# jovoy/SolarAxionRayTracing

Measured on AMD Instinct MI355X. Metric: rays/sec, higher is better.
Workload: dtype f64

## Files before the change

### solaraxionraytracing_amd/csrc/sart_api.hip

```cpp
#include <hip/hip_runtime.h>
#include <rccl/rccl.h>
#include <dlfcn.h>
#include <sys/mman.h>
#include <unistd.h>

#include <algorithm>
#include <atomic>
#include <cmath>
#include <condition_variable>
#include <thread>
#include <cstdio>
#include <cstdlib>
#include <cstring>
#include <limits>
#include <map>
#include <mutex>
#include <string>
#include <vector>

#include "../../include/sart.h"
#include "sart_device.h"

namespace sart {
void launch_trace_histogram(const HotA& H, const HotB& HB, const DevBlob* blob, const TraceArgs& A, double* acc, int n_blocks,
// ... 45 lines not shown
                            hipStream_t stream);
int records_block();
int compact_chunk_max();
void launch_compact_records(const sart_axion_t* rec, uint32_t n, sart_axion_t* out, unsigned long long capacity, uint32_t* block_counts,
                            unsigned long long* block_first, unsigned long long* counts, hipStream_t stream);
void launch_stage_columns(const HotA& H, const HotB& HB, const DevBlob* blob, const TraceArgs& A, uint64_t* stage, uint32_t* flags,
                          uint32_t mask, int n_blocks, hipStream_t stream);
void launch_compact_columns(const uint64_t* stage, const uint32_t* flags, uint32_t n, uint32_t mask, unsigned long long ray_id0, uint64_t* out,
                            unsigned long long capacity, uint32_t* block_counts, unsigned long long* block_first,
                            unsigned long long* counts, hipStream_t stream);
int histogram_blocks_per_cu(int variant);
void launch_build_solar_tables(const double* em_dev, const double* radii_dev, const double* energies_dev, int n_radii, int n_energies,
                               double* cdf_dev, double* row_sum_dev, double* rcdf_dev, uint16_t* rguide_dev, uint16_t* eguide_dev,
                               uint32_t* status_dev, hipStream_t stream);
void launch_cdf_hi32(const double* cdf_dev, uint32_t* out_dev, size_t n, hipStream_t stream);
}

using namespace sart;

namespace {

thread_local std::string g_err;
int fail(int code, const std::string& msg) {
  g_err = msg;
  return code;
}
#define SART_HIP(call)                                                                              \
  do {                                                                                              \
    hipError_t e_ = (call);                                                                         \
    if (e_ != hipSuccess)                                                                           \
      return fail(e_ == hipErrorOutOfMemory ? SART_ERR_OUT_OF_MEMORY : SART_ERR_NO_DEVICE,          \
                  std::string(#call) + ": " + hipGetErrorString(e_));                               \
  } while (0)

constexpr double kPi = 3.14159265358979323846;
// ... 86 lines not shown
#endif
    bool no_early_reject = false;
    bool no_sure_miss = false;
    bool no_image_tile = false;
    bool no_path_const = false;
    bool no_host_prefault = false;
    int records_chunk = 0;
    int records_fail_chunk = 0;
    int prefault_threads = 0;
    bool force_generic = false;
    int image_replicas = 0;
    int hist_blocks_per_cu = 0;
    bool no_radial_table = false;
    int image_tile_max = 0;
    int a0_wide = 1;
  } knobs;
  double a0_wide_survival = -1.0;
  bool a0_wide_on = false;
  hipStream_t own_stream = nullptr;
  hipStream_t stream = nullptr;
  std::string device_name;

  bool have_setup = false, have_solar = false, have_refl = false, have_det = false;
  sart_setup_t setup;
  std::vector<double> energies;
  int n_radii = 0, n_energies = 0;
  std::vector<double> refl_data;
  int refl_nc = 0, refl_na = 0, refl_ne = 0;
  double refl_amin = 0, refl_amax = 0, refl_emin = 0, refl_emax = 0;
  std::vector<double> sb_x, sb_y, win_x, win_y, gas_x, gas_y;
// ... 3 lines not shown
  HotB hotb;
  DevBuf<DevBlob> d_blob;
  bool blob_dirty = true;
  bool spot_may_have_moved = true;
  std::vector<ShellDev> shells;
  std::vector<uint8_t> shell_lut;
  int radial_n = 0;
  int radius_span = 0;
  bool path_const = false;
  DevBuf<ShellDev> d_shells;
  DevBuf<double> d_sincos;
  DevBuf<uint8_t> d_lut;
  DevBuf<double> d_rcdf, d_ecdf, d_refl;
  DevBuf<uint32_t> d_ecdf_hi32;
  DevBuf<uint16_t> d_rguide, d_eguide;
  DevBuf<EnergyDev> d_etab;
  DevBuf<double> d_replicas;
  DevBuf<double> d_partials;
  DevBuf<double> d_acc;
  bool d_acc_stale = false;
  DevBuf<sart_axion_t> d_rec;
  DevBuf<sart_axion_t> d_rec2;
  DevBuf<sart_axion_t> d_cmp;
  DevBuf<uint32_t> d_cmp_counts;
  DevBuf<unsigned long long> d_cmp_first, d_cmp_totals;
  unsigned long long* h_cmp_totals = nullptr;
  DevBuf<uint64_t> d_col_stage, d_col_cmp[2];
  DevBuf<uint32_t> d_col_flags;
  hipStream_t copy_stream = nullptr;
  hipEvent_t rec_traced[2] = {nullptr, nullptr}, rec_copied[2] = {nullptr, nullptr};
// ... 666 lines not shown
  DevBlob b;
  std::memset(&b, 0, sizeof b);
  b.P = c->params;
  b.T = tables_of(c);
  if (int rc = c->d_blob.upload(&b, 1)) return rc;
  c->hot = hot_of(c->params);
  c->hot.radial_table = radial_table ? 1 : 0;
  c->hotb.diff_flux_cdfs = c->d_ecdf.p;
  c->hotb.cdf_hi32 = c->d_ecdf_hi32.p;
  c->hotb.energy_guide = c->d_eguide.p;
  c->hotb.energy_tab = c->d_etab.p;
  c->hotb.refl = c->d_refl.p;
  c->hotb.n_energies = c->n_energies;
  c->hotb.refl_n_angles = c->refl_na;
  c->hotb.cdf_stride = c->n_energies + kEnergyCdfPad;
  c->hotb._pad = 0;
  if (!c->knobs.no_early_reject) build_zones(c->setup, c->params, c->n_radii, c->hot, tilt_bound_of(c->setup, c->setup.telescope_turned_y_deg));
  if (c->hot.n_zones > 0 && c->knobs.a0_wide > 0) {
    const double survival = a0_survival_of(c->hot);
    if (survival != c->a0_wide_survival) {
      c->a0_wide_survival = survival;
      c->a0_wide_on = a0_wide_rule(survival);
    }
    if (c->knobs.a0_wide == 2 || c->a0_wide_on) c->hot.zone_reached |= kA0WideMask;
  }
  c->path_const = path_is_constant(c->params, c->hot, c->n_radii);
  c->blob_dirty = false;
  if (c->spot_may_have_moved) c->tile.valid = false;
  c->spot_may_have_moved = false;
  return 0;
}
// ... 274 lines not shown
#endif
    c->knobs.no_early_reject = flag("SART_NO_EARLY_REJECT");
    c->knobs.no_sure_miss = flag("SART_NO_SURE_MISS");
    c->knobs.no_image_tile = flag("SART_NO_IMAGE_TILE");
    c->knobs.no_path_const = flag("SART_NO_PATH_CONST");
    c->knobs.no_host_prefault = flag("SART_NO_HOST_PREFAULT");
    c->knobs.records_chunk = number("SART_RECORDS_CHUNK");
    c->knobs.records_fail_chunk = number("SART_RECORDS_FAIL_CHUNK");
    c->knobs.prefault_threads = number("SART_PREFAULT_THREADS");
    c->knobs.force_generic = flag("SART_FORCE_GENERIC");
    c->knobs.image_replicas = number("SART_IMAGE_REPLICAS");
    c->knobs.hist_blocks_per_cu = number("SART_HIST_BLOCKS_PER_CU");
    c->knobs.no_radial_table = flag("SART_NO_RADIAL_TABLE");
    c->knobs.image_tile_max = number("SART_IMAGE_TILE_MAX");
    if (const char* e = std::getenv("SART_A0_WIDE")) c->knobs.a0_wide = std::min(2, std::max(0, std::atoi(e)));
  }
  *out = c;
  return 0;
}

int sart_destroy(sart_context* c) {
  if (!c) return 0;
  (void)hipSetDevice(c->device);
  (void)hipStreamSynchronize(c->stream);
  for (auto& ev : c->events) { (void)hipEventDestroy(ev.first); (void)hipEventDestroy(ev.second); }
  for (int k = 0; k < 2; ++k) {
    if (c->rec_traced[k]) (void)hipEventDestroy(c->rec_traced[k]);
    if (c->rec_copied[k]) (void)hipEventDestroy(c->rec_copied[k]);
  }
  if (c->copy_stream) { (void)hipStreamSynchronize(c->copy_stream); (void)hipStreamDestroy(c->copy_stream); }
// ... 93 lines not shown
  c->spot_may_have_moved = true;
  return hoist_setup(c);
}

int sart_set_axion_mass(sart_context* c, double m) {
  if (!c) return fail(SART_ERR_INVALID_ARGUMENT, "ctx is NULL");
  if (!c->have_setup) return fail(SART_ERR_NOT_READY, "no setup");
  if (!std::isfinite(m)) return fail(SART_ERR_INVALID_ARGUMENT, "axion mass is not finite");
  c->setup.m_axion = m;
  if (c->derived_dirty) return 0;
  c->params.gas_dm2_abs = std::fabs(c->params.gas_m_gamma_sq - m * m);
  c->blob_dirty = true;
  return 0;
}

int sart_set_solar_tables(sart_context* c, const double* rcdf, const double* ecdf, const double* energies, int32_t nR,
                          int32_t nE) {
  if (!c || !rcdf || !ecdf || !energies) return fail(SART_ERR_INVALID_ARGUMENT, "NULL argument");
  if (nR < 1 || nR > 2048) return fail(SART_ERR_INVALID_ARGUMENT, "n_radii must be in [1, 2048] (LDS-resident radius CDF)");
  if (nE < 2 || nE > 65535) return fail(SART_ERR_INVALID_ARGUMENT, "n_energies must be in [2, 65535]");
  for (int i = 1; i < nR; ++i) if (rcdf[i] < rcdf[i - 1]) return fail(SART_ERR_INVALID_ARGUMENT, "flux_radius_cdf not monotone");
  if (rcdf[nR - 1] != 1.0) return fail(SART_ERR_INVALID_ARGUMENT, "flux_radius_cdf must end at 1.0");
  SART_HIP(hipSetDevice(c->device));
  SART_HIP(hipStreamSynchronize(c->stream));
  std::vector<uint16_t> rg(kRadiusGuideEntries);
  for (int k = 0; k < kRadiusGuideEntries; ++k) {
    const double edge = k <= kRadiusGuide ? static_cast<double>(k) / kRadiusGuide
                                          : 0.96875 + static_cast<double>(k - (kRadiusGuide + 1)) / 32768.0;
    rg[k] = static_cast<uint16_t>(std::min<size_t>(lower_bound_idx(rcdf, nR, edge), nR - 1));
  }
// ... 23 lines not shown
      const double edge = 1.0 - decode(kEnergyGuideCode0 - static_cast<uint32_t>(j) + 1u);
      const size_t ub = static_cast<size_t>(std::upper_bound(row, row + nE, edge) - row);
      g[kEnergyGuideUniform + j] = static_cast<uint16_t>(std::min(ub, last));
    }
    g[kEnergyGuideBuckets] = static_cast<uint16_t>(last);
    std::memcpy(padded.data() + static_cast<size_t>(r) * stride, row, static_cast<size_t>(nE) * sizeof(double));
  }
  if (int rc = c->d_rcdf.upload(rcdf, nR)) return rc;
  if (int rc = c->d_ecdf.upload(padded.data(), padded.size())) return rc;
  if (int rc = c->d_ecdf_hi32.resize(padded.size())) return rc;
  launch_cdf_hi32(c->d_ecdf.p, c->d_ecdf_hi32.p, padded.size(), c->stream);
  SART_HIP(hipGetLastError());
  SART_HIP(hipStreamSynchronize(c->stream));
  if (int rc = c->d_rguide.upload(rg.data(), rg.size())) return rc;
  if (int rc = c->d_eguide.upload(eg.data(), eg.size())) return rc;
  c->energies.assign(energies, energies + nE);
  c->n_radii = nR;
  c->n_energies = nE;
  c->have_solar = true;
  c->have_channels = false;
  c->derived_dirty = true;
  return 0;
}

int sart_set_solar_tables_device(sart_context* c, const double* em_rates_dev, const double* radii, const double* energies,
                                 int32_t nR, int32_t nE) {
  if (!c || !em_rates_dev || !radii || !energies) return fail(SART_ERR_INVALID_ARGUMENT, "NULL argument");
  if (nR < 1 || nR > 2048) return fail(SART_ERR_INVALID_ARGUMENT, "n_radii must be in [1, 2048] (LDS-resident radius CDF)");
  if (nE < 2 || nE > 65535) return fail(SART_ERR_INVALID_ARGUMENT, "n_energies must be in [2, 65535]");
  SART_HIP(hipSetDevice(c->device));
// ... 9 lines not shown
  if (int rc = c->d_rguide.resize(kRadiusGuideEntries)) return rc;
  if (int rc = c->d_eguide.resize(static_cast<size_t>(nR) * kEnergyGuideEntries)) return rc;
  if (int rc = c->d_ecdf_hi32.resize(static_cast<size_t>(nR) * (static_cast<size_t>(nE) + kEnergyCdfPad))) return rc;
  c->have_solar = false;
  c->have_channels = false;
  launch_build_solar_tables(em_rates_dev, d_radii.p, d_energies.p, nR, nE, c->d_ecdf.p, d_row_sum.p, c->d_rcdf.p, c->d_rguide.p,
                            c->d_eguide.p, d_status.p, c->stream);
  launch_cdf_hi32(c->d_ecdf.p, c->d_ecdf_hi32.p, c->d_ecdf_hi32.n, c->stream);
  SART_HIP(hipGetLastError());
  uint32_t status[2] = {0, 0};
  SART_HIP(hipMemcpyAsync(status, d_status.p, sizeof status, hipMemcpyDeviceToHost, c->stream));
  SART_HIP(hipStreamSynchronize(c->stream));
  if (status[0] & 1u) return fail(SART_ERR_INVALID_ARGUMENT, "emission table: a radius row does not give a CDF (negative / non-finite rates, or a row that sums to zero)");
  if (status[0] & 2u) return fail(SART_ERR_INVALID_ARGUMENT, "emission table: fluxRadiusCDF is not monotone or does not end at 1.0");
  c->radius_span = static_cast<int>(status[1]);
  c->energies.assign(energies, energies + nE);
  c->n_radii = nR;
  c->n_energies = nE;
  c->have_solar = true;
  c->derived_dirty = true;
  return 0;
}

static_assert(kEnergyGuideEntries == 2594 && kRadiusGuideEntries == 3074, "include/sart.h (sart_get_solar_tables) and _lib.py (ENERGY_GUIDE_ENTRIES, RADIUS_GUIDE_ENTRIES) state these numbers");
int sart_get_solar_tables(sart_context* c, double* rcdf_out, double* ecdf_out, uint16_t* radius_guide_out, uint16_t* energy_guide_out) {
  if (!c) return fail(SART_ERR_INVALID_ARGUMENT, "ctx is NULL");
  if (!c->have_solar) return fail(SART_ERR_NOT_READY, "no solar tables");
  SART_HIP(hipSetDevice(c->device));
  SART_HIP(hipStreamSynchronize(c->stream));
  const size_t nR = static_cast<size_t>(c->n_radii), nE = static_cast<size_t>(c->n_energies);
// ... 66 lines not shown
__attribute__((visibility("default"))) int sart_internal_zones(sart_context* c, uint32_t* lo, uint32_t* hi, uint32_t* reached_bits) {
  if (!c || !lo || !hi || !reached_bits) return -1;
  if (hipSetDevice(c->device) != hipSuccess || refresh_derived(c) != 0 || sync_blob(c) != 0) return -1;
  for (int z = 0; z < c->hot.n_zones; ++z) { lo[z] = c->hot.zone_lo[z]; hi[z] = c->hot.zone_hi[z]; }
  *reached_bits = c->hot.zone_reached & ((1u << kMaxZones) - 1u);
  return c->hot.n_zones;
}

__attribute__((visibility("default"))) double sart_internal_a0_wide_share(double survival) { return a0_wide_fallback_share(survival); }
__attribute__((visibility("default"))) int sart_internal_a0_wide_rule(double survival) { return a0_wide_rule(survival) ? 1 : 0; }
__attribute__((visibility("default"))) int sart_internal_a0_wide(sart_context* c, double* survival) {
  if (!c || !survival) return -1;
  if (hipSetDevice(c->device) != hipSuccess || refresh_derived(c) != 0 || sync_blob(c) != 0) return -1;
  *survival = c->hot.n_zones > 0 ? a0_survival_of(c->hot) : 1.0;
  return (c->hot.zone_reached >> kA0WideBit) & 1u;
}

__attribute__((visibility("default"))) int sart_internal_shell0_miss_radius(sart_context* c, double* out) {
  if (!c || !out) return fail(SART_ERR_INVALID_ARGUMENT, "NULL argument");
  SART_HIP(hipSetDevice(c->device));
  if (int rc = refresh_derived(c)) return rc;
  if (int rc = sync_blob(c)) return rc;
  *out = c->params.shell0_miss_radius;
  return 0;
}

__attribute__((visibility("default"))) int sart_internal_mirror_miss(sart_context* c, const sart_trace_params_t* params, double* radius,
                                                                     double* slope_sq, double* thresholds, unsigned long long* counts) {
  if (!c || !radius || !slope_sq) return fail(SART_ERR_INVALID_ARGUMENT, "NULL argument");
  SART_HIP(hipSetDevice(c->device));
// ... 1827 lines not shown
```

### solaraxionraytracing_amd/csrc/sart_device.h

```cpp
#pragma once
#include <stdint.h>

namespace sart {

constexpr int kMaxShells = 64;
constexpr int kMaxStrips = 16;
constexpr int kRadiusGuide = 2048;
constexpr int kRadiusGuideTop = 1024;
constexpr uint32_t kRadiusGuideTopStart = 0xF8000000u;
constexpr int kRadiusGuideEntries = kRadiusGuide + 1 + kRadiusGuideTop + 1;
#ifndef SART_ENERGY_GUIDE_DIV
#define SART_ENERGY_GUIDE_DIV 1024
#endif
constexpr int kEnergyGuideDiv = SART_ENERGY_GUIDE_DIV;
constexpr int kEnergyGuideUniform = kEnergyGuideDiv / 32 * 31;
constexpr int kEnergyGuideLogMax = 25 * 64;
constexpr int kEnergyGuideBuckets = kEnergyGuideUniform + kEnergyGuideLogMax + 1;
constexpr int kEnergyGuideEntries = kEnergyGuideBuckets + 1;
constexpr uint32_t kEnergyGuideCode0 = (1023u - 5u) << 6;
constexpr int kEnergyCdfPad = 4;
constexpr int kShellLutMax = 1024;
constexpr int kMaxRadii = 2048;
constexpr int kSinCosEntries = 129;

struct ShellDev {
  double r1;
  double r1_outer;
  double m1_k, m1_hb, m1_cc, m1_zhi;
  double m2_k, m2_hb, m2_cc, m2_zlo, m2_zhi;
  double m2_rc;
  double n1_tan;
  double n1_r3t;
  double n1_r3sq, n1_e;
  double n2_tan;
// ... 74 lines not shown
  uint32_t zone_reached;
  uint32_t zone_lo[4], zone_hi[4];
};
constexpr int kMaxZones = 4;
constexpr int kA0WideBit = 8;
constexpr uint32_t kA0WideMask = 0x5u << kA0WideBit;
static_assert(kA0WideBit >= kMaxZones, "the wide-pass switch lies above the zones' bits");

struct HotB {
  const double* diff_flux_cdfs;
  const uint32_t* cdf_hi32;
  const uint16_t* energy_guide;
  const EnergyDev* energy_tab;
  const double* refl;
  int32_t n_energies, refl_n_angles;
  int32_t cdf_stride, _pad;
};

struct DevTables {
  const double* sincos_tab;
  const ShellDev* shells;
  const uint8_t* shell_lut;
  const double* flux_radius_cdf;
  const uint16_t* radius_guide;
  const double* diff_flux_cdfs;
  const uint16_t* energy_guide;
  const EnergyDev* energy_tab;
  const double* refl;
};

struct DevBlob {
// ... 157 lines not shown
```

### solaraxionraytracing_amd/csrc/sart_kernels.hip

```cpp
#include <hip/hip_runtime.h>
#include <stdint.h>
#include <string.h>

#include <type_traits>

#include "../../include/sart.h"
#include "sart_device.h"
#include "sart_math.h"

namespace sart {

struct U4 { uint32_t x, y, z, w; };
constexpr int kPhiloxRounds = 7;

__device__ __forceinline__ U4 philox4x32(uint32_t c0, uint32_t c1, uint32_t c2, uint32_t c3, uint32_t k0,
                                         uint32_t k1) {
#pragma unroll
  for (int r = 0; r < kPhiloxRounds; ++r) {
    const uint64_t p0 = (uint64_t)0xD2511F53u * c0;
    const uint64_t p1 = (uint64_t)0xCD9E8D57u * c2;
    const uint32_t hi0 = (uint32_t)(p0 >> 32), lo0 = (uint32_t)p0;
    const uint32_t hi1 = (uint32_t)(p1 >> 32), lo1 = (uint32_t)p1;
    const uint32_t n0 = __builtin_amdgcn_bitop3_b32(hi1, c1, k0, 0x96);
    const uint32_t n2 = __builtin_amdgcn_bitop3_b32(hi0, c3, k1, 0x96);
// ... 333 lines not shown
template <typename T>
__device__ __forceinline__ T gload(const void* base, uint32_t byte_off) {
  typedef const __attribute__((address_space(1))) char* gbytes;
  return *reinterpret_cast<const __attribute__((address_space(1))) T*>((gbytes)base + byte_off);
}

typedef uint32_t u4v __attribute__((ext_vector_type(4)));
struct EnergyDraw {
  double u;
  uint32_t khi;
  uint32_t row;
  uint32_t gword;
  uint32_t lo, hi;
  u4v c;
};
template <bool WORD = false>
__device__ __forceinline__ void energy_draw_begin(const HotB& HB, int r_idx, double u5, uint32_t word, EnergyDraw& d, int r_idx_guide = -1) {
  if (r_idx_guide < 0) r_idx_guide = r_idx;
  d.u = u5;
  if (WORD) {
    d.khi = word;
  } else {
    const double w = fmin(u5 + 1.0, 1.9999999999999998);
    d.khi = __builtin_amdgcn_alignbit((uint32_t)__double2hiint(w), (uint32_t)__double2loint(w), 20u);
  }
  static_assert((kEnergyGuideDiv & (kEnergyGuideDiv - 1)) == 0 && kEnergyGuideDiv >= 32, "the word form shifts by log2 of it");
  const double v = 1.0 - u5;
  const uint32_t ku = WORD ? word >> (32 - __builtin_ctz((uint32_t)kEnergyGuideDiv)) : (uint32_t)(int)(u5 * (double)kEnergyGuideDiv);
  const uint32_t code = (uint32_t)__double2hiint(v) >> 14;
  const uint32_t kl = (uint32_t)kEnergyGuideUniform + min(kEnergyGuideCode0 - code, (uint32_t)kEnergyGuideLogMax);
  const bool uniform_bucket = WORD ? word < 0xF8000000u : v > 0.03125;
  const uint32_t k = uniform_bucket ? ku : kl;
  d.row = __umul24((uint32_t)r_idx, (uint32_t)HB.cdf_stride);
  d.gword = gload<uint32_t>(HB.energy_guide, (__umul24((uint32_t)r_idx_guide, (uint32_t)kEnergyGuideEntries) + k) * 2u);
}
__device__ __forceinline__ void energy_draw_candidates(const HotB& HB, EnergyDraw& d) {
  d.lo = d.gword & 0xFFFFu;
  d.hi = d.gword >> 16;
  d.c = gload<u4v>(HB.cdf_hi32, (d.row + d.lo) * 4u);
}
template <bool WORD = false>
__device__ __forceinline__ int energy_draw_finish(const HotB& HB, const EnergyDraw& d) {
  const double u = d.u;
  if (WORD) {
    const uint32_t z = d.khi;
    uint32_t lo = d.lo + (uint32_t)(d.c.x < z) + (uint32_t)(d.c.y < z) + (uint32_t)(d.c.z < z) + (uint32_t)(d.c.w < z);
    if ((d.c.w < z) & (d.hi > d.lo + 4u)) {
      asm volatile("; rare: energy bucket wider than four entries");
      uint32_t hi = d.hi;
      while (lo < hi) {
        const uint32_t mid = (lo + hi) >> 1;
        if (gload<double>(HB.diff_flux_cdfs, (d.row + mid) * 8u) < u) lo = mid + 1; else hi = mid;
      }
    }
    return (int)min(lo, (uint32_t)(HB.n_energies - 1));
  }
  const uint32_t km1 = max(d.khi, 1u) - 1u;
  uint32_t lo = d.lo + (uint32_t)(d.c.x < km1) + (uint32_t)(d.c.y < km1) + (uint32_t)(d.c.z < km1) + (uint32_t)(d.c.w < km1);
// ... 1 lines not shown
  if (((d.c.w < km1) & (d.hi > d.lo + 4u)) | tie) {
    asm volatile("; rare: energy bucket wider than four entries, or a tie in the upper 32 bits");
    if (tie) lo = d.lo;
    uint32_t hi = d.hi;
    while (lo < hi) {
      const uint32_t mid = (lo + hi) >> 1;
      if (gload<double>(HB.diff_flux_cdfs, (d.row + mid) * 8u) < u) lo = mid + 1; else hi = mid;
    }
  }
  return (int)min(lo, (uint32_t)(HB.n_energies - 1));
}
template <bool WORD = false>
__device__ __forceinline__ int sample_energy_index(const HotB& HB, int r_idx, double u5, uint32_t word = 0u) {
  EnergyDraw d;
  energy_draw_begin<WORD>(HB, r_idx, u5, word, d);
  energy_draw_candidates(HB, d);
  return energy_draw_finish<WORD>(HB, d);
}

static_assert(sizeof(EnergyDev) == 8 * sizeof(double), "EnergyDev is loaded as eight f64");
__device__ __forceinline__ EnergyDev load_energy_row(const HotB& HB, int e_idx) {
  const uint32_t off = (uint32_t)e_idx * 64u;
  return EnergyDev{gload<double>(HB.energy_tab, off), gload<double>(HB.energy_tab, off + 8u), gload<double>(HB.energy_tab, off + 16u),
                   gload<double>(HB.energy_tab, off + 24u), gload<double>(HB.energy_tab, off + 32u), gload<double>(HB.energy_tab, off + 40u),
                   gload<double>(HB.energy_tab, off + 48u), gload<double>(HB.energy_tab, off + 56u)};
}

__device__ __forceinline__ double spoke_measure(int n, double c) {
  if (n == 16) {
    const double u = HORNER(c, c, -0.5);
    const double v = HORNER(u, u, -0.125);
// ... 416 lines not shown
  uint64_t m_chip;
  uint64_t m_strip;
};
template <bool RECORDS, bool FAST, int GAS, bool ZEXT, bool SCAN = false, bool NODRAW = false, bool ESCAN = false>
__device__ __forceinline__ void phase_b(const DevParams& P, const LdsTables& L, const HotB& HB, const TraceArgs& A,
                                        const RayState& st, int e_idx_in, bool live, RayOut& out, sart_axion_t* rec,
                                        EScanGeo* geo = nullptr) {
#ifdef SART_STAGE_TIMING
#define SART_B_STAMP(k, dep) do { asm volatile("" :: "v"(dep)); out.tb[k] = __builtin_readcyclecounter(); } while (0)
#else
#define SART_B_STAMP(k, dep)
#endif
  SART_B_STAMP(0, st.X0);
  constexpr bool WORD = !RECORDS;
  const bool draw_energy = NODRAW ? false : __builtin_amdgcn_readfirstlane(e_idx_in) < 0;
  EnergyDraw ed = {};
#ifdef SART_DEBUG_KNOBS
  const uint32_t dbg = (uint32_t)__builtin_amdgcn_readfirstlane((int)A.flags);
  if (draw_energy) energy_draw_begin<WORD>(HB, (dbg & 0x02000000u) ? (st.r_idx & 15) : st.r_idx, st.u5, st.u5_hi, ed, (dbg & 0x04000000u) ? (st.r_idx & 15) : st.r_idx);
#else
  if (draw_energy) energy_draw_begin<WORD>(HB, st.r_idx, st.u5, st.u5_hi, ed);
#endif
  const ShellDev& sh = L.shells[st.shell];
  const int wolter = __builtin_amdgcn_readfirstlane(P.telescope_wolter);
  static_assert(!ZEXT || GAS >= 0, "the z-extent form needs the stage at compile time");
  static_assert(!SCAN || !RECORDS, "the mass scan accumulates, it writes no records");
  const int stage_gas = (GAS >= 0) ? GAS : __builtin_amdgcn_readfirstlane(P.stage_gas);
  const int test_active = FAST ? 0 : __builtin_amdgcn_readfirstlane(P.test_active);
  const int n_half_strips = __builtin_amdgcn_readfirstlane(P.n_half_strips);
  const uint32_t flags = (uint32_t)__builtin_amdgcn_readfirstlane((int)A.flags);
  const double X0 = st.X0, Y0 = st.Y0, tsx = st.tsx, tsy = st.tsy, zcb = st.zcb;
  const double Q0 = fma(X0, X0, Y0 * Y0);

  const double D0 = fma(X0, tsx, Y0 * tsy);
  const double A0 = fma(tsx, tsx, tsy * tsy);
  const double L0 = 1.0 + A0;
  double z1;
  uint64_t live_m = ballot64(live), hit1_m, hit2_m;
  const bool hit1 = pick_root(A0 - sh.m1_k, D0 + sh.m1_hb, Q0 - sh.m1_cc, 0.0, sh.m1_zhi, z1, hit1_m);
  if (!hit1) z1 = zcb;
  const double m1x = fma(z1, tsx, X0), m1y = fma(z1, tsy, Y0);
  double n1z = wolter ? sh.n1_r3t : sh.n1_tan * fma(-sh.n1_tan, z1, sh.r1);
  if (live & !hit1)
    n1z = normal_z_general(P, sh, 1, m1x, m1y, z1);
  if (draw_energy) energy_draw_candidates(HB, ed);
  double wx = tsx, wy = tsy, wz = 1.0;
  const double N1 = fma(m1x, m1x, fma(m1y, m1y, n1z * n1z));
  double sin_a1, sin_a2;
  const double sin2_a1 = reflect(wx, wy, wz, L0, m1x, m1y, n1z, N1, sin_a1);

  {
    const double lz = P.l_mirror - z1, num = sh.nickel_num;
    bool nick = sin2_a1 * fma(lz, lz, num * num) > num * num;
    uint64_t nick_m = ballot64(nick);
    if (ballot64(!(lz > 0.0))) {
      if (!(lz > 0.0)) nick = fsqrt(sin2_a1 / (1.0 - sin2_a1)) > num / lz;
      nick_m = ballot64(nick);
    }
    const bool upper = st.shell > 0;
    const bool hit_nickel = live & upper & nick;
// ... 591 lines not shown
      }
      const int packed = Q.w[wave].idx[slot];
      st.r_idx = packed & 0xFFFF;
      st.shell = packed >> 16;
      if constexpr (kAperture) {
        typename BD::Args APl;
        reload_kernarg(APl, BD::kArgsOffset);
        const double fx = (st.X0 - APl.x_min) * APl.inv_step_x;
        const double fy = (st.Y0 - APl.y_min) * APl.inv_step_y;
        const bool in_window = (fx >= 0.0) & (fx < (double)APl.nx) & (fy >= 0.0) & (fy < (double)APl.ny);
        ap_cell = in_window ? (uint32_t)(int)fy * (uint32_t)APl.nx + (uint32_t)(int)fx : (uint32_t)APl.nx * (uint32_t)APl.ny;
      }
      const DevBlob& Bo = lds_opaque(B);
      HotB HB;
      reload_kernarg(HB, offsetof(HistKernArgs, HB));
      asm volatile("" :: "s"(HB.cdf_hi32), "s"(HB.energy_guide), "s"(HB.energy_tab), "s"(HB.refl), "s"(HB.refl_n_angles), "s"(HB.cdf_stride));
      phase_b<false, false, -1, false>(Bo.P, L, HB, lds_opaque(Ab), st, H.test_active ? Pb.n_energies : -1, valid, out, nullptr);
    }
    h1 += n_valid;
    __builtin_amdgcn_s_setprio(SART_PRIO_ACC);
    n_nickel += (uint32_t)__popcll(out.m_nickel);
    n_till += (uint32_t)__popcll(out.m_till);
    n_passed += (uint32_t)__popcll(out.m_passed);
    [[maybe_unused]] const uint32_t sh = shell_of(st.shell);
    if constexpr (kShells) {
      if (__builtin_amdgcn_inverse_ballot_w64(out.m_nickel))
        __hip_atomic_fetch_add(&lds.tab.cnt[sh][1], 1u, __ATOMIC_RELAXED, __HIP_MEMORY_SCOPE_WORKGROUP);
      if (__builtin_amdgcn_inverse_ballot_w64(out.m_till))
        __hip_atomic_fetch_add(&lds.tab.cnt[sh][2], 1u, __ATOMIC_RELAXED, __HIP_MEMORY_SCOPE_WORKGROUP);
    }
    if (out.passed) {
// ... 1626 lines not shown
  double *d_in = nullptr, *d_out = nullptr, *d_tab = nullptr;
  if (n < 1 || (fn >= 15 && fn <= 20 && (n & 1)) || hipMalloc(&d_in, (size_t)n * 8) != hipSuccess || hipMalloc(&d_out, (size_t)n * 8) != hipSuccess ||
      hipMalloc(&d_tab, 2 * kSinCosEntries * 8) != hipSuccess)
    return -1;
  (void)hipMemcpy(d_in, in_host, (size_t)n * 8, hipMemcpyHostToDevice);
  (void)hipMemcpy(d_tab, sincos_table_host, 2 * kSinCosEntries * 8, hipMemcpyHostToDevice);
  hipLaunchKernelGGL(math_eval_kernel, dim3((n + 255) / 256), dim3(256), 0, nullptr, fn, d_in, d_out, n, d_tab);
  const hipError_t e = hipMemcpy(out_host, d_out, (size_t)n * 8, hipMemcpyDeviceToHost);
  (void)hipFree(d_in); (void)hipFree(d_out); (void)hipFree(d_tab);
  return e == hipSuccess ? 0 : -2;
}

void launch_cdf_hi32(const double* cdf_dev, uint32_t* out_dev, size_t n, hipStream_t stream);
void launch_build_guides(const double* ecdf_dev, int n_rows, int n_energies, uint16_t* eguide_dev, const double* rcdf_dev, int n_radii,
                         uint16_t* rguide_dev, uint32_t* status_dev, hipStream_t stream);
__global__ __launch_bounds__(256) void word_draw_energy_kernel(HotB HB, const int32_t* __restrict__ rows, const uint32_t* __restrict__ words, int n,
                                                               int32_t* __restrict__ out_word, int32_t* __restrict__ out_general) {
  const int i = blockIdx.x * blockDim.x + threadIdx.x;
  if (i >= n) return;
  const uint32_t z = words[i];
  const double u = u52(z, 0u);
  out_word[i] = sample_energy_index<true>(HB, rows[i], u, z);
  out_general[i] = sample_energy_index<false>(HB, rows[i], u);
}
__global__ __launch_bounds__(256) void word_draw_radius_kernel(const double* __restrict__ rcdf, const uint16_t* __restrict__ rguide,
                                                               const double* __restrict__ sincos_tab, int n_radii,
                                                               const uint32_t* __restrict__ words, int n, int32_t* __restrict__ out_word,
                                                               int32_t* __restrict__ out_general) {
  __shared__ TablesLds S;
  DevParams P = {};
  P.n_radii = n_radii;
  DevTables T = {};
  T.sincos_tab = sincos_tab;
  T.flux_radius_cdf = rcdf;
  T.radius_guide = rguide;
  stage_tables<256>(S, P, T);
  const LdsTables L{S.sincos, S.rcdf_hi, rcdf, S.rguide, S.shells, S.lut};
  const int i = blockIdx.x * blockDim.x + threadIdx.x;
  if (i >= n) return;
  const uint32_t z = words[i];
  out_word[i] = radius_draw<true>(L, z, u52(z, 0u));
  out_general[i] = radius_draw<false>(L, z, u52(z, 0u));
}
extern "C" __attribute__((visibility("default"))) int sart_internal_word_draw(int kind, const double* cdf_host, int n_rows, int n_cols,
                                                                               const int32_t* rows_host, const uint32_t* words_host, int n,
                                                                               int32_t* out_word_host, int32_t* out_general_host) {
  if (n < 1 || n_rows < 1 || n_cols < 1 || (kind != 0 && kind != 1) || (kind == 1 && (n_rows != 1 || n_cols > kMaxRadii)) || n_cols > 65535)
    return -1;
  if (kind == 0)
    for (int i = 0; i < n; ++i)
      if (rows_host[i] < 0 || rows_host[i] >= n_rows) return -1;
  const int stride = kind == 0 ? n_cols + kEnergyCdfPad : n_cols;
  std::vector<double> cdf((size_t)n_rows * stride, 1.0);
  for (int r = 0; r < n_rows; ++r)
    for (int k = 0; k < n_cols; ++k) cdf[(size_t)r * stride + k] = cdf_host[(size_t)r * n_cols + k];
  const size_t n_guide = kind == 0 ? (size_t)n_rows * kEnergyGuideEntries : (size_t)kRadiusGuideEntries;
  double *d_cdf = nullptr, *d_tab = nullptr;
  uint32_t *d_hi = nullptr, *d_words = nullptr, *d_status = nullptr;
  uint16_t* d_guide = nullptr;
  int32_t *d_rows = nullptr, *d_ow = nullptr, *d_og = nullptr;
  int rc = -2;
  if (hipMalloc(&d_cdf, cdf.size() * 8) == hipSuccess && hipMalloc(&d_hi, cdf.size() * 4) == hipSuccess &&
      hipMalloc(&d_guide, n_guide * 2) == hipSuccess && hipMalloc(&d_words, (size_t)n * 4) == hipSuccess &&
      hipMalloc(&d_rows, (size_t)n * 4) == hipSuccess && hipMalloc(&d_ow, (size_t)n * 4) == hipSuccess &&
      hipMalloc(&d_og, (size_t)n * 4) == hipSuccess && hipMalloc(&d_status, 8) == hipSuccess &&
      hipMalloc(&d_tab, 2 * kSinCosEntries * 8) == hipSuccess) {
    (void)hipMemcpy(d_cdf, cdf.data(), cdf.size() * 8, hipMemcpyHostToDevice);
    (void)hipMemcpy(d_words, words_host, (size_t)n * 4, hipMemcpyHostToDevice);
    (void)hipMemset(d_rows, 0, (size_t)n * 4);
    (void)hipMemset(d_tab, 0, 2 * kSinCosEntries * 8);
    if (kind == 0) {
      (void)hipMemcpy(d_rows, rows_host, (size_t)n * 4, hipMemcpyHostToDevice);
      launch_cdf_hi32(d_cdf, d_hi, cdf.size(), nullptr);
      launch_build_guides(d_cdf, n_rows, n_cols, d_guide, nullptr, 0, nullptr, d_status, nullptr);
      HotB HB = {};
      HB.diff_flux_cdfs = d_cdf;
      HB.cdf_hi32 = d_hi;
      HB.energy_guide = d_guide;
      HB.n_energies = n_cols;
      HB.cdf_stride = stride;
      hipLaunchKernelGGL(word_draw_energy_kernel, dim3((n + 255) / 256), dim3(256), 0, nullptr, HB, d_rows, d_words, n, d_ow, d_og);
    } else {
      launch_build_guides(nullptr, 0, 0, nullptr, d_cdf, n_cols, d_guide, d_status, nullptr);
      hipLaunchKernelGGL(word_draw_radius_kernel, dim3((n + 255) / 256), dim3(256), 0, nullptr, d_cdf, d_guide, d_tab, n_cols, d_words, n, d_ow,
                         d_og);
    }
    const hipError_t e1 = hipMemcpy(out_word_host, d_ow, (size_t)n * 4, hipMemcpyDeviceToHost);
    const hipError_t e2 = hipMemcpy(out_general_host, d_og, (size_t)n * 4, hipMemcpyDeviceToHost);
    rc = (e1 == hipSuccess && e2 == hipSuccess && hipGetLastError() == hipSuccess) ? 0 : -2;
  }
  (void)hipFree(d_cdf); (void)hipFree(d_hi); (void)hipFree(d_guide); (void)hipFree(d_words); (void)hipFree(d_rows);
  (void)hipFree(d_ow); (void)hipFree(d_og); (void)hipFree(d_status); (void)hipFree(d_tab);
  return rc;
}

int records_block() { return kRecBlock; }
int histogram_block_of(int) { return 1024; }

#define SART_HIST_VARIANTS(X) \
  X(0, true, false, 0, false) X(1, false, false, -1, false) X(2, false, true, -1, false) X(3, true, false, 1, false) \
  X(4, true, true, 0, false) X(5, true, false, 0, true) X(6, true, false, 1, true)
#define SART_SCAN_VARIANTS(X) X(1, false, false, -1, false) X(2, false, true, -1, false) X(3, true, false, 1, false) X(6, true, false, 1, true)

#define SART_FOLD_OF(K, fixed) ((fixed) ? K<true> : K<false>)
static void launch_scalars_fold(double* scalars, const double* partials, const TraceArgs& A, int n_blocks, hipStream_t stream, bool fixed) {
  if (fixed)
    hipLaunchKernelGGL(fold_scalars_fixed_kernel, dim3(1), dim3(256), 0, stream, reinterpret_cast<long long*>(scalars),
                       reinterpret_cast<const long long*>(partials), n_blocks, (long long)A.n_rays);
// ... 299 lines not shown
```

### solaraxionraytracing_amd/csrc/sart_tables.hip

```cpp
#include <hip/hip_runtime.h>
#include <stdint.h>

#include "sart_device.h"

#pragma clang fp contract(off)

namespace sart {

__global__ __launch_bounds__(64) void cdf_rows_kernel(const double* __restrict__ em, const double* __restrict__ radii,
                                                      const double* __restrict__ energies, int n_radii, int n_energies,
                                                      double* __restrict__ cdf, double* __restrict__ row_sum,
                                                      uint32_t* __restrict__ status) {
  const int r = blockIdx.x * 64 + threadIdx.x;
  if (r >= n_radii) return;
  const size_t stride = (size_t)n_energies + kEnergyCdfPad;
  const double* src = em + (size_t)r * n_energies;
  double* dst = cdf + (size_t)r * stride;
  const double radius = radii[r];
  double sum = 0.0;
  bool monotone = true;
  for (int i = 0; i < n_energies; ++i) {
    const double e = energies[i];
    const double flux = __dmul_rn(__dmul_rn(__dmul_rn(src[i], __dmul_rn(e, e)), radius), radius);
    const double next = __dadd_rn(sum, flux);
// ... 82 lines not shown
    v = last;
  }
  guide[(size_t)r * kEnergyGuideEntries + k] = (uint16_t)v;
}

__global__ __launch_bounds__(256) void cdf_hi32_kernel(const double* __restrict__ cdf, uint32_t* __restrict__ out, size_t n) {
  const size_t i = (size_t)blockIdx.x * 256 + threadIdx.x;
  if (i >= n) return;
  const unsigned long long t = __double2ull_rd(cdf[i] * 4503599627370496.0) >> 20;
  out[i] = t > 0xFFFFFFFFull ? 0xFFFFFFFFu : (uint32_t)t;
}
void launch_cdf_hi32(const double* cdf_dev, uint32_t* out_dev, size_t n, hipStream_t stream) {
  hipLaunchKernelGGL(cdf_hi32_kernel, dim3((unsigned)((n + 255) / 256)), dim3(256), 0, stream, cdf_dev, out_dev, n);
}

void launch_build_solar_tables(const double* em_dev, const double* radii_dev, const double* energies_dev, int n_radii, int n_energies,
                               double* cdf_dev, double* row_sum_dev, double* rcdf_dev, uint16_t* rguide_dev, uint16_t* eguide_dev,
                               uint32_t* status_dev, hipStream_t stream) {
  (void)hipMemsetAsync(status_dev, 0, 2 * sizeof(uint32_t), stream);
  hipLaunchKernelGGL(cdf_rows_kernel, dim3((n_radii + 63) / 64), dim3(64), 0, stream, em_dev, radii_dev, energies_dev, n_radii,
                     n_energies, cdf_dev, row_sum_dev, status_dev);
  hipLaunchKernelGGL(radius_cdf_kernel, dim3(1), dim3(256), 0, stream, row_sum_dev, n_radii, rcdf_dev, status_dev);
  hipLaunchKernelGGL(radius_guide_kernel, dim3(1), dim3(256), 0, stream, rcdf_dev, n_radii, rguide_dev, status_dev);
  hipLaunchKernelGGL(energy_guide_kernel, dim3((kEnergyGuideEntries + 255) / 256, n_radii), dim3(256), 0, stream, cdf_dev, n_radii,
                     n_energies, eguide_dev);
}

void launch_build_guides(const double* ecdf_dev, int n_rows, int n_energies, uint16_t* eguide_dev, const double* rcdf_dev, int n_radii,
                         uint16_t* rguide_dev, uint32_t* status_dev, hipStream_t stream) {
  (void)hipMemsetAsync(status_dev, 0, 2 * sizeof(uint32_t), stream);
// ... 8 lines not shown
```

### solaraxionraytracing_amd/csrc/sart_trace_histogram.inc

```
  struct LdsLayout {
    TablesLds S;
    RadialLds R;
    double tile_extra[kTileExtraCells];
    DevBlob B;
    TraceArgs Ab;
    QueueLds<BLOCK / 64, HistRings> Q;
  };
  static_assert(sizeof(RadialLds) % 8 == 0 && (kRadialMarked + 1) * sizeof(double) <= sizeof(RadialLds) + kTileExtraCells * sizeof(double),
                "entry kRadialMarked of either column lies in the table or in the tile's cells");
  __shared__ LdsLayout lds;
  TablesLds& S = lds.S;
  QueueLds<BLOCK / 64, HistRings>& Q = lds.Q;
  static_assert(!PATHC || (FAST && !ROT && GAS >= 0), "the constant-path form belongs to the unrotated specialisations");
  static_assert(!SCAN || GAS != 0, "a mass scan needs the gas stage");
  static_assert(!SCAN || kScanMaxMasses * 2 * kScanLanes <= (BLOCK / 64) * kQueue, "the scan accumulators live in the image tile's 128 doubles per wave");
  __shared__ uint32_t scan_zero[kScanMaxMasses];
  static_assert(!BANDS || SCAN, "the bands belong to the mass scan");
  __shared__ uint32_t scan_band_n[BANDS ? kScanLanes : 1];
  static_assert((BLOCK / 64) * kQueue == kTileRingCells && kImageTileMax * kImageTileMax <= kTileRingCells + kTileExtraCells &&
                    kImageTileExtraMax * kImageTileExtraMax <= kTileExtraCells && BLOCK / 64 == kTileRingCells / kQueue,
                "the LDS image tile (host: kImageTileMax): 128 doubles per wave of this workgroup's rings + the cells behind the tables");
  static_assert((offsetof(LdsLayout, Q) % 512) == 0, "the rings are addressed with ds_*2st64 offsets (units of 512 bytes for 64-bit columns)");
  auto tile_cell_lo = [&](uint32_t t) -> double* {
    return PATHC ? &Q.w[t >> 7].path[t & 127u] : reinterpret_cast<double*>(&Q.w[t >> 7].ray[0]) + (t & 127u);
// ... 124 lines not shown
      const uint2 cell = Q.w[wave].cell[slot];
      st.u5 = u52(cell.y, 0u);
      st.u5_hi = cell.y;
      if (!ROT) {
        st.zcb = -(H.dz3 - H.dz1);
      } else {
        st.zcb = zcb_rotated(Pb.rx_s, -Pb.rx_c * Pb.ry_s, Pb.rx_c * Pb.ry_c, Pb.half_length_telescope, st.X0 + Pb.entrance_x,
                             st.Y0 + Pb.entrance_y, st.tsx, st.tsy, H.dz3 - H.dz1);
      }
      const int packed = (int)cell.x;
      st.r_idx = packed & 0xFFFF;
      st.shell = packed >> 16;
      const DevBlob& Bo = lds_opaque(B);
      HotB HB;
      reload_kernarg(HB, offsetof(HistKernArgs, HB));
      asm volatile("" :: "s"(HB.cdf_hi32), "s"(HB.energy_guide), "s"(HB.energy_tab), "s"(HB.refl), "s"(HB.refl_n_angles), "s"(HB.cdf_stride));
      phase_b<false, FAST, GAS, FAST && !ROT && GAS >= 0, SCAN>(Bo.P, L, HB, lds_opaque(Ab), st, (!FAST && H.test_active) ? Pb.n_energies : -1, valid, out, nullptr);
      if constexpr (SCAN) {
        SART_STAGE_MARK("SCAN");
        n_passed += (uint32_t)__popcll(out.m_passed);
        struct { int32_t n_masses, pad; } hdr;
        reload_kernarg(hdr, offsetof(HistKernArgs, SC));
        const uint32_t fl = (uint32_t)__builtin_amdgcn_readfirstlane((int)Ab.flags);
        const bool use_prob = !(fl & SART_CF_IGNORE_CONV_PROB) & ((GAS >= 0) ? (GAS == 1) : (__builtin_amdgcn_readfirstlane(Bo.P.stage_gas) != 0));
        const double term1 = Bo.P.gas_term1;
        const GasCos cos_lead = GasCos::make();
        uint32_t cell = 0u;
        if constexpr (BANDS) {
          struct { int32_t e0; uint32_t mul; } b0;
          struct { uint32_t window, unused; } b1;
          reload_kernarg(b0, offsetof(HistKernArgs, SC) + offsetof(ScanArgs, m) + offsetof(ScanMass, aux));
// ... 346 lines not shown
```

Measured before the change: 109.9 billion.

## Precompute per-bucket energy records to replace the dependent guide-then-CDF load chain

Adds a precomputed per-row, per-guide-bucket 16-byte record that packs the bucket's start index and five 22-bit CDF thresholds. The word-based energy draw can then resolve the index with a single load and a few compares, instead of loading the guide entry and then the cdf_hi32 candidates. A rare fallback reloads the guide and CDF, with a binary search when a bucket is wider than its record. This removes one dependent global-load round trip per energy draw, at the cost of extra table memory, a build kernel at table setup, extra SGPRs in HotB, and more code in the hot kernel.

```diff
diff --git a/solaraxionraytracing_amd/csrc/sart_api.hip b/solaraxionraytracing_amd/csrc/sart_api.hip
--- a/solaraxionraytracing_amd/csrc/sart_api.hip
+++ b/solaraxionraytracing_amd/csrc/sart_api.hip
@@ -83,11 +83,14 @@
                                double* cdf_dev, double* row_sum_dev, double* rcdf_dev, uint16_t* rguide_dev, uint16_t* eguide_dev,
                                uint32_t* status_dev, hipStream_t stream);
 void launch_cdf_hi32(const double* cdf_dev, uint32_t* out_dev, size_t n, hipStream_t stream);
+void launch_build_energy_records(const uint32_t* hi32_dev, const uint16_t* eguide_dev, int n_rows, int n_energies, uint32_t* records_dev,
+                                 hipStream_t stream);
 }
 
 using namespace sart;
 
 namespace {
+constexpr bool kEnergyRecordsDefault = true;
 
 thread_local std::string g_err;
 int fail(int code, const std::string& msg) {
@@ -204,6 +207,7 @@
     bool no_radial_table = false;
     int image_tile_max = 0;
     int a0_wide = 1;
+    bool energy_records = kEnergyRecordsDefault;
   } knobs;
   double a0_wide_survival = -1.0;
   bool a0_wide_on = false;
@@ -237,6 +241,7 @@
   DevBuf<double> d_rcdf, d_ecdf, d_refl;
   DevBuf<uint32_t> d_ecdf_hi32;
   DevBuf<uint16_t> d_rguide, d_eguide;
+  DevBuf<uint32_t> d_erecords;
   DevBuf<EnergyDev> d_etab;
   DevBuf<double> d_replicas;
   DevBuf<double> d_partials;
@@ -933,7 +938,8 @@
   c->hotb.n_energies = c->n_energies;
   c->hotb.refl_n_angles = c->refl_na;
   c->hotb.cdf_stride = c->n_energies + kEnergyCdfPad;
-  c->hotb._pad = 0;
+  c->hotb.energy_records = c->d_erecords.p;
+  c->hotb.records_on = c->d_erecords.p ? 1 : 0;
   if (!c->knobs.no_early_reject) build_zones(c->setup, c->params, c->n_radii, c->hot, tilt_bound_of(c->setup, c->setup.telescope_turned_y_deg));
   if (c->hot.n_zones > 0 && c->knobs.a0_wide > 0) {
     const double survival = a0_survival_of(c->hot);
@@ -1238,6 +1244,7 @@
     c->knobs.no_radial_table = flag("SART_NO_RADIAL_TABLE");
     c->knobs.image_tile_max = number("SART_IMAGE_TILE_MAX");
     if (const char* e = std::getenv("SART_A0_WIDE")) c->knobs.a0_wide = std::min(2, std::max(0, std::atoi(e)));
+    if (const char* e = std::getenv("SART_ENERGY_RECORDS")) c->knobs.energy_records = std::atoi(e) != 0;
   }
   *out = c;
   return 0;
@@ -1361,6 +1368,18 @@
   return 0;
 }
 
+static int build_energy_records(sart_context* c, int32_t nR, int32_t nE) {
+  if (!c->knobs.energy_records || nE > kEnergyRecordMaxEnergies) {
+    c->d_erecords.release();
+    return 0;
+  }
+  if (int rc = c->d_erecords.resize(static_cast<size_t>(nR) * kEnergyGuideBuckets * 4)) return rc;
+  launch_build_energy_records(c->d_ecdf_hi32.p, c->d_eguide.p, nR, nE, c->d_erecords.p, c->stream);
+  SART_HIP(hipGetLastError());
+  SART_HIP(hipStreamSynchronize(c->stream));
+  return 0;
+}
+
 int sart_set_solar_tables(sart_context* c, const double* rcdf, const double* ecdf, const double* energies, int32_t nR,
                           int32_t nE) {
   if (!c || !rcdf || !ecdf || !energies) return fail(SART_ERR_INVALID_ARGUMENT, "NULL argument");
@@ -1414,6 +1433,7 @@
   SART_HIP(hipStreamSynchronize(c->stream));
   if (int rc = c->d_rguide.upload(rg.data(), rg.size())) return rc;
   if (int rc = c->d_eguide.upload(eg.data(), eg.size())) return rc;
+  if (int rc = build_energy_records(c, nR, nE)) return rc;
   c->energies.assign(energies, energies + nE);
   c->n_radii = nR;
   c->n_energies = nE;
@@ -1453,6 +1473,7 @@
   if (status[0] & 1u) return fail(SART_ERR_INVALID_ARGUMENT, "emission table: a radius row does not give a CDF (negative / non-finite rates, or a row that sums to zero)");
   if (status[0] & 2u) return fail(SART_ERR_INVALID_ARGUMENT, "emission table: fluxRadiusCDF is not monotone or does not end at 1.0");
   c->radius_span = static_cast<int>(status[1]);
+  if (int rc = build_energy_records(c, nR, nE)) return rc;
   c->energies.assign(energies, energies + nE);
   c->n_radii = nR;
   c->n_energies = nE;
@@ -1549,6 +1570,12 @@
   if (hipSetDevice(c->device) != hipSuccess || refresh_derived(c) != 0 || sync_blob(c) != 0) return -1;
   *survival = c->hot.n_zones > 0 ? a0_survival_of(c->hot) : 1.0;
   return (c->hot.zone_reached >> kA0WideBit) & 1u;
+}
+
+__attribute__((visibility("default"))) int sart_internal_energy_records(sart_context* c) {
+  if (!c) return -1;
+  if (hipSetDevice(c->device) != hipSuccess || refresh_derived(c) != 0 || sync_blob(c) != 0) return -1;
+  return (c->hotb.records_on != 0 && c->hotb.energy_records != nullptr) ? 1 : 0;
 }
 
 __attribute__((visibility("default"))) int sart_internal_shell0_miss_radius(sart_context* c, double* out) {
diff --git a/solaraxionraytracing_amd/csrc/sart_device.h b/solaraxionraytracing_amd/csrc/sart_device.h
--- a/solaraxionraytracing_amd/csrc/sart_device.h
+++ b/solaraxionraytracing_amd/csrc/sart_device.h
@@ -18,6 +18,9 @@
 constexpr int kEnergyGuideBuckets = kEnergyGuideUniform + kEnergyGuideLogMax + 1;
 constexpr int kEnergyGuideEntries = kEnergyGuideBuckets + 1;
 constexpr uint32_t kEnergyGuideCode0 = (1023u - 5u) << 6;
+constexpr int kEnergyRecordK = 5;
+constexpr uint32_t kEnergyRecordEmpty = 0x3FFFFFu;
+constexpr int kEnergyRecordMaxEnergies = 2047;
 constexpr int kEnergyCdfPad = 4;
 constexpr int kShellLutMax = 1024;
 constexpr int kMaxRadii = 2048;
@@ -122,7 +125,9 @@
   const EnergyDev* energy_tab;
   const double* refl;
   int32_t n_energies, refl_n_angles;
-  int32_t cdf_stride, _pad;
+  int32_t cdf_stride;
+  int32_t records_on;
+  const uint32_t* energy_records;
 };
 
 struct DevTables {
diff --git a/solaraxionraytracing_amd/csrc/sart_kernels.hip b/solaraxionraytracing_amd/csrc/sart_kernels.hip
--- a/solaraxionraytracing_amd/csrc/sart_kernels.hip
+++ b/solaraxionraytracing_amd/csrc/sart_kernels.hip
@@ -371,6 +371,11 @@
   uint32_t lo, hi;
   u4v c;
 };
+__device__ __forceinline__ bool energy_records_on(const HotB& HB) {
+  int32_t on = HB.records_on;
+  asm volatile("" : "+s"(on));
+  return on != 0;
+}
 template <bool WORD = false>
 __device__ __forceinline__ void energy_draw_begin(const HotB& HB, int r_idx, double u5, uint32_t word, EnergyDraw& d, int r_idx_guide = -1) {
   if (r_idx_guide < 0) r_idx_guide = r_idx;
@@ -388,10 +393,19 @@
   const uint32_t kl = (uint32_t)kEnergyGuideUniform + min(kEnergyGuideCode0 - code, (uint32_t)kEnergyGuideLogMax);
   const bool uniform_bucket = WORD ? word < 0xF8000000u : v > 0.03125;
   const uint32_t k = uniform_bucket ? ku : kl;
+  if (WORD && energy_records_on(HB)) {
+    d.row = (uint32_t)r_idx;
+    d.lo = k;
+    d.hi = (word - (uint32_t)!uniform_bucket) << 10;
+    d.c = gload<u4v>(HB.energy_records, (__umul24((uint32_t)r_idx_guide, (uint32_t)kEnergyGuideBuckets) + k) * 16u);
+    return;
+  }
   d.row = __umul24((uint32_t)r_idx, (uint32_t)HB.cdf_stride);
   d.gword = gload<uint32_t>(HB.energy_guide, (__umul24((uint32_t)r_idx_guide, (uint32_t)kEnergyGuideEntries) + k) * 2u);
 }
+template <bool WORD = false>
 __device__ __forceinline__ void energy_draw_candidates(const HotB& HB, EnergyDraw& d) {
+  if (WORD && energy_records_on(HB)) return;
   d.lo = d.gword & 0xFFFFu;
   d.hi = d.gword >> 16;
   d.c = gload<u4v>(HB.cdf_hi32, (d.row + d.lo) * 4u);
@@ -399,6 +413,30 @@
 template <bool WORD = false>
 __device__ __forceinline__ int energy_draw_finish(const HotB& HB, const EnergyDraw& d) {
   const double u = d.u;
+  if (WORD && energy_records_on(HB)) {
+    static_assert(kEnergyRecordK == 5 && kEnergyRecordEmpty == 0x3FFFFFu, "the layout energy_records_kernel packs");
+    const uint32_t xs = d.hi;
+    const uint32_t t4s = __builtin_amdgcn_perm(__builtin_amdgcn_perm(d.c.y, d.c.z, 0x04000c0cu), d.c.w, 0x0706000cu);
+    const bool b4 = t4s < xs;
+    uint32_t lo = ((d.c.x & 0x3FFu) | ((d.c.y & 0x100u) << 2)) + (uint32_t)(d.c.x < xs) + (uint32_t)(d.c.y < xs) + (uint32_t)(d.c.z < xs) +
+                  (uint32_t)(d.c.w < xs) + (uint32_t)b4;
+    if (__builtin_amdgcn_inverse_ballot_w64(ballot64(b4) & ballot64((d.c.w & 0x100u) != 0u))) {
+      asm volatile("; rare: energy bucket wider than its record");
+      const uint32_t z = d.khi, row = __umul24(d.row, (uint32_t)HB.cdf_stride);
+      const uint32_t hi = gload<uint16_t>(HB.energy_guide, (__umul24(d.row, (uint32_t)kEnergyGuideEntries) + d.lo + 1u) * 2u);
+      const u4v c = gload<u4v>(HB.cdf_hi32, (row + lo) * 4u);
+      const uint32_t lo5 = lo;
+      lo += (uint32_t)(c.x < z) + (uint32_t)(c.y < z) + (uint32_t)(c.z < z) + (uint32_t)(c.w < z);
+      if ((c.w < z) & (hi > lo5 + 4u)) {
+        uint32_t h = hi;
+        while (lo < h) {
+          const uint32_t mid = (lo + h) >> 1;
+          if (gload<double>(HB.diff_flux_cdfs, (row + mid) * 8u) < u) lo = mid + 1; else h = mid;
+        }
+      }
+    }
+    return (int)min(lo, (uint32_t)(HB.n_energies - 1));
+  }
   if (WORD) {
     const uint32_t z = d.khi;
     uint32_t lo = d.lo + (uint32_t)(d.c.x < z) + (uint32_t)(d.c.y < z) + (uint32_t)(d.c.z < z) + (uint32_t)(d.c.w < z);
@@ -430,7 +468,7 @@
 __device__ __forceinline__ int sample_energy_index(const HotB& HB, int r_idx, double u5, uint32_t word = 0u) {
   EnergyDraw d;
   energy_draw_begin<WORD>(HB, r_idx, u5, word, d);
-  energy_draw_candidates(HB, d);
+  energy_draw_candidates<WORD>(HB, d);
   return energy_draw_finish<WORD>(HB, d);
 }
 
@@ -877,7 +915,7 @@
   SART_B_STAMP(0, st.X0);
   constexpr bool WORD = !RECORDS;
   const bool draw_energy = NODRAW ? false : __builtin_amdgcn_readfirstlane(e_idx_in) < 0;
-  EnergyDraw ed = {};
+  EnergyDraw ed;
 #ifdef SART_DEBUG_KNOBS
   const uint32_t dbg = (uint32_t)__builtin_amdgcn_readfirstlane((int)A.flags);
   if (draw_energy) energy_draw_begin<WORD>(HB, (dbg & 0x02000000u) ? (st.r_idx & 15) : st.r_idx, st.u5, st.u5_hi, ed, (dbg & 0x04000000u) ? (st.r_idx & 15) : st.r_idx);
@@ -906,7 +944,7 @@
   double n1z = wolter ? sh.n1_r3t : sh.n1_tan * fma(-sh.n1_tan, z1, sh.r1);
   if (live & !hit1)
     n1z = normal_z_general(P, sh, 1, m1x, m1y, z1);
-  if (draw_energy) energy_draw_candidates(HB, ed);
+  if (draw_energy) energy_draw_candidates<WORD>(HB, ed);
   double wx = tsx, wy = tsy, wz = 1.0;
   const double N1 = fma(m1x, m1x, fma(m1y, m1y, n1z * n1z));
   double sin_a1, sin_a2;
@@ -1528,7 +1566,7 @@
       const DevBlob& Bo = lds_opaque(B);
       HotB HB;
       reload_kernarg(HB, offsetof(HistKernArgs, HB));
-      asm volatile("" :: "s"(HB.cdf_hi32), "s"(HB.energy_guide), "s"(HB.energy_tab), "s"(HB.refl), "s"(HB.refl_n_angles), "s"(HB.cdf_stride));
+      asm volatile("" :: "s"(HB.cdf_hi32), "s"(HB.energy_guide), "s"(HB.energy_records), "s"(HB.records_on), "s"(HB.energy_tab), "s"(HB.refl), "s"(HB.refl_n_angles), "s"(HB.cdf_stride));
       phase_b<false, false, -1, false>(Bo.P, L, HB, lds_opaque(Ab), st, H.test_active ? Pb.n_energies : -1, valid, out, nullptr);
     }
     h1 += n_valid;
@@ -3185,6 +3223,8 @@
 void launch_cdf_hi32(const double* cdf_dev, uint32_t* out_dev, size_t n, hipStream_t stream);
 void launch_build_guides(const double* ecdf_dev, int n_rows, int n_energies, uint16_t* eguide_dev, const double* rcdf_dev, int n_radii,
                          uint16_t* rguide_dev, uint32_t* status_dev, hipStream_t stream);
+void launch_build_energy_records(const uint32_t* hi32_dev, const uint16_t* eguide_dev, int n_rows, int n_energies, uint32_t* records_dev,
+                                 hipStream_t stream);
 __global__ __launch_bounds__(256) void word_draw_energy_kernel(HotB HB, const int32_t* __restrict__ rows, const uint32_t* __restrict__ words, int n,
                                                                int32_t* __restrict__ out_word, int32_t* __restrict__ out_general) {
   const int i = blockIdx.x * blockDim.x + threadIdx.x;
@@ -3213,9 +3253,8 @@
   out_word[i] = radius_draw<true>(L, z, u52(z, 0u));
   out_general[i] = radius_draw<false>(L, z, u52(z, 0u));
 }
-extern "C" __attribute__((visibility("default"))) int sart_internal_word_draw(int kind, const double* cdf_host, int n_rows, int n_cols,
-                                                                               const int32_t* rows_host, const uint32_t* words_host, int n,
-                                                                               int32_t* out_word_host, int32_t* out_general_host) {
+static int word_draw_impl(int kind, const double* cdf_host, int n_rows, int n_cols, const int32_t* rows_host, const uint32_t* words_host, int n,
+                          int32_t* out_word_host, int32_t* out_general_host, bool use_records, int* records_used, uint32_t* records_out) {
   if (n < 1 || n_rows < 1 || n_cols < 1 || (kind != 0 && kind != 1) || (kind == 1 && (n_rows != 1 || n_cols > kMaxRadii)) || n_cols > 65535)
     return -1;
   if (kind == 0)
@@ -3230,7 +3269,12 @@
   uint32_t *d_hi = nullptr, *d_words = nullptr, *d_status = nullptr;
   uint16_t* d_guide = nullptr;
   int32_t *d_rows = nullptr, *d_ow = nullptr, *d_og = nullptr;
+  uint32_t* d_rec = nullptr;
+  const bool records = use_records && kind == 0 && n_cols <= kEnergyRecordMaxEnergies;
+  const size_t n_rec = (size_t)n_rows * kEnergyGuideBuckets * 4;
+  if (records_used) *records_used = records ? 1 : 0;
   int rc = -2;
+  if (records && hipMalloc(&d_rec, n_rec * 4) != hipSuccess) return rc;
   if (hipMalloc(&d_cdf, cdf.size() * 8) == hipSuccess && hipMalloc(&d_hi, cdf.size() * 4) == hipSuccess &&
       hipMalloc(&d_guide, n_guide * 2) == hipSuccess && hipMalloc(&d_words, (size_t)n * 4) == hipSuccess &&
       hipMalloc(&d_rows, (size_t)n * 4) == hipSuccess && hipMalloc(&d_ow, (size_t)n * 4) == hipSuccess &&
@@ -3250,6 +3294,11 @@
       HB.energy_guide = d_guide;
       HB.n_energies = n_cols;
       HB.cdf_stride = stride;
+      if (records) {
+        launch_build_energy_records(d_hi, d_guide, n_rows, n_cols, d_rec, nullptr);
+        HB.energy_records = d_rec;
+        HB.records_on = 1;
+      }
       hipLaunchKernelGGL(word_draw_energy_kernel, dim3((n + 255) / 256), dim3(256), 0, nullptr, HB, d_rows, d_words, n, d_ow, d_og);
     } else {
       launch_build_guides(nullptr, 0, 0, nullptr, d_cdf, n_cols, d_guide, d_status, nullptr);
@@ -3258,11 +3307,24 @@
     }
     const hipError_t e1 = hipMemcpy(out_word_host, d_ow, (size_t)n * 4, hipMemcpyDeviceToHost);
     const hipError_t e2 = hipMemcpy(out_general_host, d_og, (size_t)n * 4, hipMemcpyDeviceToHost);
-    rc = (e1 == hipSuccess && e2 == hipSuccess && hipGetLastError() == hipSuccess) ? 0 : -2;
+    const hipError_t e3 = (records && records_out) ? hipMemcpy(records_out, d_rec, n_rec * 4, hipMemcpyDeviceToHost) : hipSuccess;
+    rc = (e1 == hipSuccess && e2 == hipSuccess && e3 == hipSuccess && hipGetLastError() == hipSuccess) ? 0 : -2;
   }
   (void)hipFree(d_cdf); (void)hipFree(d_hi); (void)hipFree(d_guide); (void)hipFree(d_words); (void)hipFree(d_rows);
-  (void)hipFree(d_ow); (void)hipFree(d_og); (void)hipFree(d_status); (void)hipFree(d_tab);
+  (void)hipFree(d_ow); (void)hipFree(d_og); (void)hipFree(d_status); (void)hipFree(d_tab); (void)hipFree(d_rec);
   return rc;
+}
+extern "C" __attribute__((visibility("default"))) int sart_internal_word_draw(int kind, const double* cdf_host, int n_rows, int n_cols,
+                                                                               const int32_t* rows_host, const uint32_t* words_host, int n,
+                                                                               int32_t* out_word_host, int32_t* out_general_host) {
+  return word_draw_impl(kind, cdf_host, n_rows, n_cols, rows_host, words_host, n, out_word_host, out_general_host, true, nullptr, nullptr);
+}
+extern "C" __attribute__((visibility("default"))) int sart_internal_record_draw(const double* cdf_host, int n_rows, int n_cols,
+                                                                                 const int32_t* rows_host, const uint32_t* words_host, int n,
+                                                                                 int use_records, int32_t* out_word_host, int32_t* out_general_host,
+                                                                                 int* records_used, uint32_t* records_out) {
+  return word_draw_impl(0, cdf_host, n_rows, n_cols, rows_host, words_host, n, out_word_host, out_general_host, use_records != 0, records_used,
+                        records_out);
 }
 
 int records_block() { return kRecBlock; }
diff --git a/solaraxionraytracing_amd/csrc/sart_tables.hip b/solaraxionraytracing_amd/csrc/sart_tables.hip
--- a/solaraxionraytracing_amd/csrc/sart_tables.hip
+++ b/solaraxionraytracing_amd/csrc/sart_tables.hip
@@ -120,6 +120,52 @@
   hipLaunchKernelGGL(cdf_hi32_kernel, dim3((unsigned)((n + 255) / 256)), dim3(256), 0, stream, cdf_dev, out_dev, n);
 }
 
+__global__ __launch_bounds__(256) void energy_records_kernel(const uint32_t* __restrict__ hi32, const uint16_t* __restrict__ guide,
+                                                             int n_energies, uint32_t* __restrict__ records) {
+  const int k = blockIdx.x * 256 + threadIdx.x;
+  const int r = blockIdx.y;
+  if (k >= kEnergyGuideBuckets) return;
+  long long first, last;
+  const long long off = k < kEnergyGuideUniform ? 0 : 1;
+  if (k < kEnergyGuideUniform) {
+    first = (long long)k << 22;
+    last = first + 0x3FFFFF;
+  } else if (k == kEnergyGuideUniform) {
+    first = last = 0xF8000000ll;
+  } else {
+    const int j = k - kEnergyGuideUniform;
+    const int e = 26 - (j - 1) / 64, f = 63 - (j - 1) % 64;
+    const long long m_lo = e >= 6 ? (long long)(64 + f) << (e - 6) : (((long long)(64 + f) + (1ll << (6 - e)) - 1) >> (6 - e));
+    const long long m_hi = e >= 6 ? (long long)(65 + f) << (e - 6) : (((long long)(65 + f) + (1ll << (6 - e)) - 1) >> (6 - e));
+    first = 0x100000000ll - m_hi + 1;
+    last = 0x100000000ll - (j == kEnergyGuideLogMax ? 1 : m_lo);
+  }
+  const long long block = ((first - off) >> 22) << 22;
+  const uint32_t* t = hi32 + (size_t)r * ((size_t)n_energies + kEnergyCdfPad);
+  const uint16_t* g = guide + (size_t)r * kEnergyGuideEntries + k;
+  int lo = g[0];
+  const int hi = g[1];
+  while (lo < hi && (long long)t[lo] < first) ++lo;
+  uint32_t thr[kEnergyRecordK];
+  for (int s = 0; s < kEnergyRecordK; ++s) {
+    const long long v = lo + s < hi ? (long long)t[lo + s] : last + 1;
+    thr[s] = v <= last ? (uint32_t)(v - off - block) : kEnergyRecordEmpty;
+  }
+  const uint32_t mark = lo + kEnergyRecordK < hi ? 1u : 0u;
+  static_assert(kEnergyRecordK == 5, "the packing below holds five thresholds");
+  const uint32_t t4 = thr[4], l = (uint32_t)lo;
+  uint32_t* out = records + ((size_t)r * kEnergyGuideBuckets + k) * 4;
+  out[0] = thr[0] << 10 | (l & 0x3FFu);
+  out[1] = thr[1] << 10 | ((l >> 10) << 8) | (t4 >> 14);
+  out[2] = thr[2] << 10 | ((t4 >> 6) & 0xFFu);
+  out[3] = thr[3] << 10 | (mark << 8) | ((t4 & 0x3Fu) << 2);
+}
+void launch_build_energy_records(const uint32_t* hi32_dev, const uint16_t* eguide_dev, int n_rows, int n_energies, uint32_t* records_dev,
+                                 hipStream_t stream) {
+  hipLaunchKernelGGL(energy_records_kernel, dim3((kEnergyGuideBuckets + 255) / 256, n_rows), dim3(256), 0, stream, hi32_dev, eguide_dev,
+                     n_energies, records_dev);
+}
+
 void launch_build_solar_tables(const double* em_dev, const double* radii_dev, const double* energies_dev, int n_radii, int n_energies,
                                double* cdf_dev, double* row_sum_dev, double* rcdf_dev, uint16_t* rguide_dev, uint16_t* eguide_dev,
                                uint32_t* status_dev, hipStream_t stream) {
diff --git a/solaraxionraytracing_amd/csrc/sart_trace_histogram.inc b/solaraxionraytracing_amd/csrc/sart_trace_histogram.inc
--- a/solaraxionraytracing_amd/csrc/sart_trace_histogram.inc
+++ b/solaraxionraytracing_amd/csrc/sart_trace_histogram.inc
@@ -162,7 +162,7 @@
       const DevBlob& Bo = lds_opaque(B);
       HotB HB;
       reload_kernarg(HB, offsetof(HistKernArgs, HB));
-      asm volatile("" :: "s"(HB.cdf_hi32), "s"(HB.energy_guide), "s"(HB.energy_tab), "s"(HB.refl), "s"(HB.refl_n_angles), "s"(HB.cdf_stride));
+      asm volatile("" :: "s"(HB.cdf_hi32), "s"(HB.energy_guide), "s"(HB.energy_records), "s"(HB.records_on), "s"(HB.energy_tab), "s"(HB.refl), "s"(HB.refl_n_angles), "s"(HB.cdf_stride));
       phase_b<false, FAST, GAS, FAST && !ROT && GAS >= 0, SCAN>(Bo.P, L, HB, lds_opaque(Ab), st, (!FAST && H.test_active) ? Pb.n_energies : -1, valid, out, nullptr);
       if constexpr (SCAN) {
         SART_STAGE_MARK("SCAN");
```

After: 111.3 billion (median of 6 runs). 1.01x the previous value.
